# mirams/PyHillFit

Measured on AMD Instinct MI355X. Metric: MCMC samples/sec (whole node), higher is better.
Workload: dtype f64

## Files before the change

### pyhillfit_amd/csrc/phf_model.h

```cpp
#ifndef PHF_MODEL_H
#define PHF_MODEL_H

#include "phf_math.h"
#include "phf_philox.h"

#define PHF_SIGMA_FLOOR 1e-3
#define PHF_PIC50_RATE 0.2
#define PHF_PIC50_LOWER (-3.0)
#define PHF_HILL_UPPER 10.0
#define PHF_SIGMA_LOC 1e-3
#define PHF_SIGMA_SHAPE_M1 4.0
#define PHF_SIGMA_INV_SCALE (4.0 / (6.0 - 1e-3))
#define PHF_HILL_ARG_CAP 40.0

PHF_HD double phf_hill_den(int model, double ln_conc, double hill, double ln_ic50, phf_ktab k_exp) {
  const double a = (model == 1) ? (ln_conc - ln_ic50) : hill * (ln_conc - ln_ic50);
  return 1.0 + phf_exp_capped_k(__builtin_fmin(a, PHF_HILL_ARG_CAP), k_exp);
}

PHF_HD double phf_hill_percent(double w, phf_ktab k_exp) { return phf_fma(-PHF_K100(k_exp), w, PHF_K100(k_exp)); }
#define PHF_PCT_(w_) phf_hill_percent((w_), k_exp)

PHF_HD double phf_censored_z(double pred, double y, double inv_s) {
  const double sgn = (y > 50.0) ? 1.0 : -1.0;
  return (sgn * (pred - y)) * inv_s;
}

PHF_HD void phf_sl_log_target(int model, const double* lc, const double* y, const double* w, int n_other, int n_cens,
                              double n_other_points, double ss_within, double pi_bit, double temperature,
                              const double* th, phf_ktab k_exp, phf_ktab k_log,
                              double* out_lik, double* out_prior, double* out_ll1) {
  const double pic50 = th[0];
  const double hill = (model == 1) ? 1.0 : th[1];
  const double sigma = (model == 1) ? th[1] : th[2];
  const double ln_ic50 = PHF_LN10 * (6.0 - pic50);
  const double sl = sigma - PHF_SIGMA_LOC;
  const double inv_s = phf_rcp(sigma);
  const double log_sigma = phf_log_pos_k(sigma, k_log);
  const double log_sl = phf_log_pos_k(sl, k_log);

  double sse = ss_within, cens = 0.0;
  int j = 0;
  for (; j + 4 <= n_other; j += 4) {
    const phf_ktab ke = k_exp;
    const double d0 = phf_hill_den(model, lc[j], hill, ln_ic50, ke), d1 = phf_hill_den(model, lc[j + 1], hill, ln_ic50, ke);
    const double d2 = phf_hill_den(model, lc[j + 2], hill, ln_ic50, ke), d3 = phf_hill_den(model, lc[j + 3], hill, ln_ic50, ke);
    const double p01 = d0 * d1, p23 = d2 * d3;
    const double inv = phf_rcp(p01 * p23);
    const double i01 = inv * p23, i23 = inv * p01;
    const double r0 = y[j] - PHF_PCT_(i01 * d1), r1 = y[j + 1] - PHF_PCT_(i01 * d0);
    const double r2 = y[j + 2] - PHF_PCT_(i23 * d3), r3 = y[j + 3] - PHF_PCT_(i23 * d2);
    sse = phf_fma(w[j] * r0, r0, sse); sse = phf_fma(w[j + 1] * r1, r1, sse);
    sse = phf_fma(w[j + 2] * r2, r2, sse); sse = phf_fma(w[j + 3] * r3, r3, sse);
  }
  const int rem = n_other - j;
  if (rem == 3) {
    const phf_ktab ke = k_exp;
    const double d0 = phf_hill_den(model, lc[j], hill, ln_ic50, ke), d1 = phf_hill_den(model, lc[j + 1], hill, ln_ic50, ke);
    const double d2 = phf_hill_den(model, lc[j + 2], hill, ln_ic50, ke);
    const double p01 = d0 * d1;
    const double inv = phf_rcp(p01 * d2);
    const double i01 = inv * d2;
    const double r0 = y[j] - PHF_PCT_(i01 * d1), r1 = y[j + 1] - PHF_PCT_(i01 * d0);
    const double r2 = y[j + 2] - PHF_PCT_(inv * p01);
    sse = phf_fma(w[j] * r0, r0, sse); sse = phf_fma(w[j + 1] * r1, r1, sse); sse = phf_fma(w[j + 2] * r2, r2, sse);
  } else if (rem == 2) {
    const phf_ktab ke = k_exp;
    const double d0 = phf_hill_den(model, lc[j], hill, ln_ic50, ke), d1 = phf_hill_den(model, lc[j + 1], hill, ln_ic50, ke);
    const double inv = phf_rcp(d0 * d1);
    const double r0 = y[j] - PHF_PCT_(inv * d1), r1 = y[j + 1] - PHF_PCT_(inv * d0);
    sse = phf_fma(w[j] * r0, r0, sse); sse = phf_fma(w[j + 1] * r1, r1, sse);
  } else if (rem == 1) {
    const double r = y[j] - PHF_PCT_(phf_rcp(phf_hill_den(model, lc[j], hill, ln_ic50, k_exp)));
    sse = phf_fma(w[j] * r, r, sse);
  }
  j = n_other;
  const int n = n_other + n_cens;
  for (; j + 2 <= n; j += 2) {
    const phf_ktab ke = k_exp;
    const double d0 = phf_hill_den(model, lc[j], hill, ln_ic50, ke), d1 = phf_hill_den(model, lc[j + 1], hill, ln_ic50, ke);
    const double inv = phf_rcp(d0 * d1);
    const double z0 = phf_censored_z(PHF_PCT_(inv * d1), y[j], inv_s);
    const double z1 = phf_censored_z(PHF_PCT_(inv * d0), y[j + 1], inv_s);
    cens = phf_fma(w[j], phf_log_ndtr_tab(z0, -z0 * PHF_INV_SQRT2), cens);
    cens = phf_fma(w[j + 1], phf_log_ndtr_tab(z1, -z1 * PHF_INV_SQRT2), cens);
  }
  for (; j < n; ++j) {
    const double pred = PHF_PCT_(phf_rcp(phf_hill_den(model, lc[j], hill, ln_ic50, k_exp)));
    const double z = phf_censored_z(pred, y[j], inv_s);
    cens = phf_fma(w[j], phf_log_ndtr_tab(z, -z * PHF_INV_SQRT2), cens);
  }
  double a = cens - pi_bit;
  a = phf_fma(-n_other_points, log_sigma, a);
  a = phf_fma(-sse, 0.5 * inv_s * inv_s, a);
  if (sigma <= PHF_SIGMA_FLOOR) a = -PHF_INF;
  double lik = temperature * a;
  if (temperature == 0.0) lik = 0.0;
  *out_lik = lik;
  *out_ll1 = a;

  const int outside = (pic50 < PHF_PIC50_LOWER)
                      | (sigma <= PHF_SIGMA_LOC)
                      | ((model == 2) & ((hill < 0.0) | (hill > PHF_HILL_UPPER)));
  const double g = phf_fma(PHF_SIGMA_SHAPE_M1, log_sl, -sl * PHF_SIGMA_INV_SCALE);
  const double lp = -PHF_PIC50_RATE * pic50 + g;
  *out_prior = outside ? -PHF_INF : lp;
}

#define PHF_SHARE_PUT_(jj, d_) do { if (share_mask) den_slot[(jj) * slot_stride] = (d_); } while (0)
#define PHF_CDEN_(jj) ((((share_mask) >> ((jj) - n_other)) & 1u) ? den_slot[den_off[(jj) - n_other]] \
                                                                 : phf_hill_den(model, lc[jj], hill, ln_ic50, k_exp))
PHF_HD void phf_sl_log_target_shared(int model, const double* lc, const double* y, const double* w, int n_other, int n_cens,
                                     double n_other_points, double ss_within, double pi_bit, double temperature,
                                     const double* th, phf_ktab k_exp, phf_ktab k_log,
                                     unsigned share_mask, const int* den_off, double* den_slot, int slot_stride,
                                     double* out_lik, double* out_prior, double* out_ll1) {
  const double pic50 = th[0];
  const double hill = (model == 1) ? 1.0 : th[1];
  const double sigma = (model == 1) ? th[1] : th[2];
  const double ln_ic50 = PHF_LN10 * (6.0 - pic50);
  const double sl = sigma - PHF_SIGMA_LOC;
  const double inv_s = phf_rcp(sigma);
  const double log_sigma = phf_log_pos_k(sigma, k_log);
  const double log_sl = phf_log_pos_k(sl, k_log);

  double sse = ss_within, cens = 0.0;
  int j = 0;
  for (; j + 4 <= n_other; j += 4) {
    const phf_ktab ke = k_exp;
    const double d0 = phf_hill_den(model, lc[j], hill, ln_ic50, ke), d1 = phf_hill_den(model, lc[j + 1], hill, ln_ic50, ke);
    const double d2 = phf_hill_den(model, lc[j + 2], hill, ln_ic50, ke), d3 = phf_hill_den(model, lc[j + 3], hill, ln_ic50, ke);
    PHF_SHARE_PUT_(j, d0); PHF_SHARE_PUT_(j + 1, d1); PHF_SHARE_PUT_(j + 2, d2); PHF_SHARE_PUT_(j + 3, d3);
    const double p01 = d0 * d1, p23 = d2 * d3;
    const double inv = phf_rcp(p01 * p23);
    const double i01 = inv * p23, i23 = inv * p01;
    const double r0 = y[j] - PHF_PCT_(i01 * d1), r1 = y[j + 1] - PHF_PCT_(i01 * d0);
    const double r2 = y[j + 2] - PHF_PCT_(i23 * d3), r3 = y[j + 3] - PHF_PCT_(i23 * d2);
    sse = phf_fma(w[j] * r0, r0, sse); sse = phf_fma(w[j + 1] * r1, r1, sse);
    sse = phf_fma(w[j + 2] * r2, r2, sse); sse = phf_fma(w[j + 3] * r3, r3, sse);
  }
  const int rem = n_other - j;
  if (rem == 3) {
    const phf_ktab ke = k_exp;
    const double d0 = phf_hill_den(model, lc[j], hill, ln_ic50, ke), d1 = phf_hill_den(model, lc[j + 1], hill, ln_ic50, ke);
    const double d2 = phf_hill_den(model, lc[j + 2], hill, ln_ic50, ke);
    PHF_SHARE_PUT_(j, d0); PHF_SHARE_PUT_(j + 1, d1); PHF_SHARE_PUT_(j + 2, d2);
    const double p01 = d0 * d1;
    const double inv = phf_rcp(p01 * d2);
    const double i01 = inv * d2;
    const double r0 = y[j] - PHF_PCT_(i01 * d1), r1 = y[j + 1] - PHF_PCT_(i01 * d0);
    const double r2 = y[j + 2] - PHF_PCT_(inv * p01);
    sse = phf_fma(w[j] * r0, r0, sse); sse = phf_fma(w[j + 1] * r1, r1, sse); sse = phf_fma(w[j + 2] * r2, r2, sse);
  } else if (rem == 2) {
    const phf_ktab ke = k_exp;
    const double d0 = phf_hill_den(model, lc[j], hill, ln_ic50, ke), d1 = phf_hill_den(model, lc[j + 1], hill, ln_ic50, ke);
    PHF_SHARE_PUT_(j, d0); PHF_SHARE_PUT_(j + 1, d1);
    const double inv = phf_rcp(d0 * d1);
    const double r0 = y[j] - PHF_PCT_(inv * d1), r1 = y[j + 1] - PHF_PCT_(inv * d0);
    sse = phf_fma(w[j] * r0, r0, sse); sse = phf_fma(w[j + 1] * r1, r1, sse);
  } else if (rem == 1) {
    const double d0 = phf_hill_den(model, lc[j], hill, ln_ic50, k_exp);
    PHF_SHARE_PUT_(j, d0);
    const double r = y[j] - PHF_PCT_(phf_rcp(d0));
    sse = phf_fma(w[j] * r, r, sse);
  }
  j = n_other;
  const int n = n_other + n_cens;
  for (; j + 2 <= n; j += 2) {
    const double d0 = PHF_CDEN_(j), d1 = PHF_CDEN_(j + 1);
    const double inv = phf_rcp(d0 * d1);
    const double z0 = phf_censored_z(PHF_PCT_(inv * d1), y[j], inv_s);
    const double z1 = phf_censored_z(PHF_PCT_(inv * d0), y[j + 1], inv_s);
    cens = phf_fma(w[j], phf_log_ndtr_tab(z0, -z0 * PHF_INV_SQRT2), cens);
    cens = phf_fma(w[j + 1], phf_log_ndtr_tab(z1, -z1 * PHF_INV_SQRT2), cens);
  }
  for (; j < n; ++j) {
    const double pred = PHF_PCT_(phf_rcp(PHF_CDEN_(j)));
    const double z = phf_censored_z(pred, y[j], inv_s);
    cens = phf_fma(w[j], phf_log_ndtr_tab(z, -z * PHF_INV_SQRT2), cens);
  }
  double a = cens - pi_bit;
  a = phf_fma(-n_other_points, log_sigma, a);
  a = phf_fma(-sse, 0.5 * inv_s * inv_s, a);
  if (sigma <= PHF_SIGMA_FLOOR) a = -PHF_INF;
  double lik = temperature * a;
  if (temperature == 0.0) lik = 0.0;
  *out_lik = lik;
  *out_ll1 = a;

  const int outside = (pic50 < PHF_PIC50_LOWER)
                      | (sigma <= PHF_SIGMA_LOC)
                      | ((model == 2) & ((hill < 0.0) | (hill > PHF_HILL_UPPER)));
  const double g = phf_fma(PHF_SIGMA_SHAPE_M1, log_sl, -sl * PHF_SIGMA_INV_SCALE);
  const double lp = -PHF_PIC50_RATE * pic50 + g;
  *out_prior = outside ? -PHF_INF : lp;
}
#undef PHF_SHARE_PUT_
#undef PHF_CDEN_

PHF_HD double phf_sl_log_prior(int model, const double* th, phf_ktab k_log) {
  const double pic50 = th[0];
  const double hill = (model == 1) ? 1.0 : th[1];
  const double sigma = (model == 1) ? th[1] : th[2];
  const double sl = sigma - PHF_SIGMA_LOC;
  const double log_sl = phf_log_pos_k(sl, k_log);
  const int outside = (pic50 < PHF_PIC50_LOWER)
                      | (sigma <= PHF_SIGMA_LOC)
                      | ((model == 2) & ((hill < 0.0) | (hill > PHF_HILL_UPPER)));
  const double g = phf_fma(PHF_SIGMA_SHAPE_M1, log_sl, -sl * PHF_SIGMA_INV_SCALE);
  const double lp = -PHF_PIC50_RATE * pic50 + g;
  return outside ? -PHF_INF : lp;
}

PHF_HD double phf_mh_draws(int d, uint32_t chain_id, uint32_t problem_id, uint32_t t, uint32_t seed_lo,
                           uint32_t seed_hi, phf_ktab k_log, double* z) {
  const phf_u32x4 b = phf_philox_mh(chain_id, problem_id, t, 0u, seed_lo, seed_hi);
  z[0] = phf_normal_u32(b.w[0]);
  z[1] = phf_normal_u32(b.w[1]);
  if (d == 2) {
    z[2] = 0.0;
    const double u = phf_uniform53(b.w[2], b.w[3]);
    const double log_u = phf_log_pos_k(u, k_log);
    return (u < PHF_DBL_MIN) ? -PHF_INF : log_u;
  }
  z[2] = phf_normal_u32(b.w[2]);
  return phf_log_pos_k(phf_unit_open32(b.w[3]), k_log);
}

PHF_HD uint32_t phf_mh_draws_w3(uint32_t chain_id, uint32_t problem_id, uint32_t t, uint32_t seed_lo, uint32_t seed_hi, double* z) {
  const phf_u32x4 b = phf_philox_mh(chain_id, problem_id, t, 0u, seed_lo, seed_hi);
  z[0] = phf_normal_u32(b.w[0]);
  z[1] = phf_normal_u32(b.w[1]);
  z[2] = phf_normal_u32(b.w[2]);
  return b.w[3];
}

#define PHF_ACCEPT_U32_BAND 0x1p18f
PHF_HD int phf_mh_accept_u32(double x, uint32_t w, phf_ktab k_log) {
#if defined(__HIP_DEVICE_COMPILE__)
  const float t = __builtin_amdgcn_exp2f(__builtin_fmaf((float)x, 0x1.715476p+0f, 32.0f));
  const float dw = (float)w - t;
  bool acc = dw < 0.0f;
  if (PHF_ANY_LANE(__builtin_fabsf(dw) <= PHF_ACCEPT_U32_BAND)) {
    const bool exact = phf_log_pos_k(phf_unit_open32(w), k_log) < x;
    acc = (__builtin_fabsf(dw) <= PHF_ACCEPT_U32_BAND) ? exact : acc;
  }
  return acc;
#else
  return phf_log_pos_k(phf_unit_open32(w), k_log) < x;
#endif
}

#endif
```

### pyhillfit_amd/csrc/phf_single_level.hip

```cpp
#include <hip/hip_runtime.h>

#include "../../include/pyhillfit_amd.h"
#include "phf_common.h"
#include "phf_hier3_isa.h"
#include "phf_model.h"

namespace {

constexpr int kBlock = 64;
thread_local int g_last_sl_kernel = 0;
constexpr int kQueuePoison = 0x40000000;
constexpr int kQueueMaxRounds = 16;
constexpr int kDenSlots = 4;
constexpr int kMaxShared = 4;

template <int MODEL> struct Dim { static constexpr int d = (MODEL == 1) ? 2 : 3; };

#ifndef PHF_CHOL_FUSED_PIVOT
#define PHF_CHOL_FUSED_PIVOT 1
#endif
template <int D>
__device__ __forceinline__ void chol_packed(const double* c, double* l) {
  double inv[D];
#pragma unroll
  for (int i = 0; i < D; ++i) {
#pragma unroll
    for (int j = 0; j <= i; ++j) {
      double s = c[i * (i + 1) / 2 + j];
#pragma unroll
      for (int k = 0; k < j; ++k) s = phf_fma(-l[i * (i + 1) / 2 + k], l[j * (j + 1) / 2 + k], s);
      if (i == j) {
        const bool pos = s > 0.0;
        double ir = 0.0;
#if PHF_CHOL_FUSED_PIVOT
        const double rs = (i + 1 < D) ? phf_sqrt_rcp_pos(s, &ir) : phf_sqrt_pos(s);
#else
        const double rs = phf_sqrt_pos(s);
        ir = phf_rcp(rs);
#endif
        const double r = pos ? rs : 0.0;
        l[i * (i + 1) / 2 + i] = r;
        inv[i] = pos ? ir : 0.0;
      } else {
        l[i * (i + 1) / 2 + j] = s * inv[j];
      }
    }
  }
}

struct AdvanceArgs {
  phf_points pts;
  phf_problems prob;
  phf_mh_config cfg;
  int64_t t_begin, t_end;
  double* state;
  double* rows;
  double* moments;
  int64_t moments_after;
  int32_t blocks_per_problem;
  int32_t* queue;
  int32_t quantum;
};

__device__ __forceinline__ void stage_points(const phf_points& pts, int pair, double* s_pts, int& n_other,
                                             int& n_zero, int& n_hundred) {
  const int32_t* cnt = pts.counts + 4 * pair;
  n_other = cnt[0]; n_zero = cnt[1]; n_hundred = cnt[2];
  const int n = n_other + n_zero + n_hundred;
  for (int j = threadIdx.x; j < n; j += kBlock) {
    s_pts[j] = pts.ln_conc[(size_t)pair * pts.stride + j];
    s_pts[pts.stride + j] = pts.response[(size_t)pair * pts.stride + j];
    s_pts[2 * pts.stride + j] = pts.weight[(size_t)pair * pts.stride + j];
  }
  __syncthreads();
}

template <int MODEL, bool MOMENTS, int KO, int KC, unsigned SHARE, bool LONE_WAVE>
__device__ __forceinline__ void advance_body(const AdvanceArgs& a, const double* s_pts, double* s_den, const int* den_off, int q,
                                             int c, int pair, int n_other_rt, int n_cens_rt, const int64_t t_begin, const int64_t t_end) {
  static_assert(SHARE == 0 || (KO >= 1 && KO <= kDenSlots && KC >= 1 && KC <= kMaxShared && (SHARE >> KC) == 0),
                "shared denominators need a straight-line body with at most kDenSlots uncensored entries");
  constexpr int D = Dim<MODEL>::d;
  constexpr int NTRI = D * (D + 1) / 2;
  const int C = a.prob.chains_per_problem;
  const int n_other = (KO >= 0) ? KO : n_other_rt;
  const int n_cens = (KC >= 0) ? KC : n_cens_rt;
  const double* lc = s_pts;
  const double* yv = s_pts + a.pts.stride;
  const double* wv = s_pts + 2 * a.pts.stride;
  const double pi_bit = a.pts.pi_bit[pair];
  const double n_other_points = a.pts.extra[2 * pair], ss_within = a.pts.extra[2 * pair + 1];
  const double temperature = a.prob.temperature[q];
  const uint32_t pid = a.prob.problem_id[q];
  const uint32_t cid = a.prob.chain_id_base + (a.prob.chain_offset ? a.prob.chain_offset[q] : 0u) + (uint32_t)c;
  uint32_t seed_lo = (uint32_t)a.cfg.seed, seed_hi = (uint32_t)(a.cfg.seed >> 32);
  if (!LONE_WAVE) { asm volatile("" : "+v"(seed_lo)); asm volatile("" : "+v"(seed_hi)); }
  const size_t nchains = (size_t)a.prob.num_problems * C;
  const size_t g = (size_t)q * C + c;

  double th[D], mean[D], cov[NTRI], L[NTRI];
  double* sp = a.state + g;
#pragma unroll
  for (int i = 0; i < D; ++i) th[i] = sp[(size_t)i * nchains];
  double lt = sp[(size_t)D * nchains];
#pragma unroll
  for (int i = 0; i < D; ++i) mean[i] = sp[(size_t)(D + 1 + i) * nchains];
#pragma unroll
  for (int i = 0; i < NTRI; ++i) cov[i] = sp[(size_t)(2 * D + 1 + i) * nchains];
  double loga = sp[(size_t)(2 * D + 1 + NTRI) * nchains];
  double nacc = sp[(size_t)(2 * D + 2 + NTRI) * nchains];
  double ll1 = sp[(size_t)(2 * D + 3 + NTRI) * nchains];
  PHF_KFETCH_V(k_exp, phf_k_exp, PHF_K_EXP_N);
  PHF_KFETCH_V(k_log, phf_k_log, PHF_K_LOG_N);
  chol_packed<D>(cov, L);
  double sc = phf_exp_fast_k(0.5 * loga, k_exp);

  double m1[D + 1], m2[D + 1], mll = 0.0;
  constexpr bool want_moments = MOMENTS;
  if (want_moments) {
#pragma unroll
    for (int i = 0; i <= D; ++i) {
      m1[i] = a.moments[(size_t)i * nchains + g];
      m2[i] = a.moments[(size_t)(D + 1 + i) * nchains + g];
    }
    mll = a.moments[(size_t)(2 * D + 2) * nchains + g];
  }

  const int thin = a.cfg.thinning;
  int until_save = thin - (int)(t_begin % thin);
  const bool save_rows = a.rows != nullptr;
  const size_t row_stride = (size_t)a.prob.num_problems * (D + 1) * C;
  double* out = a.rows + ((size_t)q * (D + 1)) * C + c + (size_t)(t_begin / thin - a.t_begin / thin) * row_stride;

  double z[3];
  double log_u = 0.0;
  uint32_t w_u = 0u;
  if constexpr (D == 3) w_u = phf_mh_draws_w3(cid, pid, (uint32_t)(t_begin + 1), seed_lo, seed_hi, z);
  else log_u = phf_mh_draws(D, cid, pid, (uint32_t)(t_begin + 1), seed_lo, seed_hi, k_log, z);
  const bool reset_mean = a.cfg.reset_mean_at_adapt_start != 0;
  for (int64_t t = t_begin + 1; t <= t_end; ++t) {
    double star[D];
#pragma unroll
    for (int i = 0; i < D; ++i) {
      double v = L[i * (i + 1) / 2 + i] * z[i];
#pragma unroll
      for (int k = i - 1; k >= 0; --k) v = phf_fma(L[i * (i + 1) / 2 + k], z[k], v);
      star[i] = phf_fma(sc, v, th[i]);
    }
    double lik_star, prior_star, ll1_star;
    phf_sl_log_target_shared(MODEL, lc, yv, wv, n_other, n_cens, n_other_points, ss_within, pi_bit, temperature, star, k_exp, k_log,
                             SHARE, den_off, s_den + threadIdx.x, kBlock, &lik_star, &prior_star, &ll1_star);
    const double lt_star = lik_star + prior_star;
    const bool acc = (D == 3) ? (bool)phf_mh_accept_u32(lt_star - lt, w_u, k_log) : log_u < lt_star - lt;
    if (acc) {
#pragma unroll
      for (int i = 0; i < D; ++i) th[i] = star[i];
      lt = lt_star;
      ll1 = ll1_star;
    }
    nacc += acc ? 1.0 : 0.0;
    const bool adapting = t > a.cfg.adapt_start;
    const bool reset_now = reset_mean && t == a.cfg.adapt_start;
    const double gs_tab = a.cfg.gamma[adapting ? t - a.cfg.adapt_start : 0];
    const double gs = adapting ? gs_tab : 0.0;
    const double omg = 1.0 - gs;
    const double gm = reset_now ? 1.0 : gs, omm = reset_now ? 0.0 : omg;
    {
      double v[D];
#pragma unroll
      for (int i = 0; i < D; ++i) v[i] = th[i] - mean[i];
#pragma unroll
      for (int i = 0; i < D; ++i)
#pragma unroll
        for (int j = 0; j <= i; ++j)
          cov[i * (i + 1) / 2 + j] = phf_fma(gs, v[i] * v[j], omg * cov[i * (i + 1) / 2 + j]);
#pragma unroll
      for (int i = 0; i < D; ++i) mean[i] = phf_fma(gm, th[i], omm * mean[i]);
      loga = phf_fma(gs, acc ? 0.75 : -0.25, loga);
    }
    double z_next[3];
    double log_u_next = 0.0;
    uint32_t w_u_next = 0u;
    if constexpr (D == 3) w_u_next = phf_mh_draws_w3(cid, pid, (uint32_t)(t + 1), seed_lo, seed_hi, z_next);
    else log_u_next = phf_mh_draws(D, cid, pid, (uint32_t)(t + 1), seed_lo, seed_hi, k_log, z_next);
    chol_packed<D>(cov, L);
    sc = phf_exp_fast_k(0.5 * loga, k_exp);
#pragma unroll
    for (int i = 0; i < 3; ++i) z[i] = z_next[i];
    log_u = log_u_next;
    w_u = w_u_next;
    if (--until_save == 0) {
      until_save = thin;
      if (save_rows) {
#pragma unroll
        for (int i = 0; i < D; ++i) out[(size_t)i * C] = th[i];
        out[(size_t)D * C] = lt;
        out += row_stride;
      }
      if (want_moments && t > a.moments_after) {
#pragma unroll
        for (int i = 0; i < D; ++i) { m1[i] += th[i]; m2[i] = phf_fma(th[i], th[i], m2[i]); }
        m1[D] += lt; m2[D] = phf_fma(lt, lt, m2[D]);
        mll += ll1;
      }
    }
  }

#pragma unroll
  for (int i = 0; i < D; ++i) sp[(size_t)i * nchains] = th[i];
  sp[(size_t)D * nchains] = lt;
#pragma unroll
  for (int i = 0; i < D; ++i) sp[(size_t)(D + 1 + i) * nchains] = mean[i];
#pragma unroll
  for (int i = 0; i < NTRI; ++i) sp[(size_t)(2 * D + 1 + i) * nchains] = cov[i];
  sp[(size_t)(2 * D + 1 + NTRI) * nchains] = loga;
  sp[(size_t)(2 * D + 2 + NTRI) * nchains] = nacc;
  sp[(size_t)(2 * D + 3 + NTRI) * nchains] = ll1;
  if (want_moments) {
#pragma unroll
    for (int i = 0; i <= D; ++i) {
      a.moments[(size_t)i * nchains + g] = m1[i];
      a.moments[(size_t)(D + 1 + i) * nchains + g] = m2[i];
    }
    a.moments[(size_t)(2 * D + 2) * nchains + g] = mll;
  }
}

#define PHF_BODY_(ko, kc, sh) \
  advance_body<MODEL, MOMENTS, ko, kc, sh, WPS == 1>(a, s_pts, s_den, den_off, q, c, pair, n_other, n_cens, t_begin, t_end)
#define PHF_SHAPE_CASE(ko, kc) case (ko) * 8 + (kc): PHF_BODY_(ko, kc, 0u); break;
#define PHF_SHAPE_CASE_SHARED(ko, kc, sh) \
  case (ko) * 8 + (kc): if ((share & (sh)) == (sh)) PHF_BODY_(ko, kc, sh); else PHF_BODY_(ko, kc, 0u); break;
#define PHF_SHAPE_ROW(ko) PHF_SHAPE_CASE(ko, 0) PHF_SHAPE_CASE(ko, 1) PHF_SHAPE_CASE(ko, 2) PHF_SHAPE_CASE(ko, 3) PHF_SHAPE_CASE(ko, 4)

__device__ __forceinline__ unsigned share_map(const double* s_pts, int n_other, int n_cens, int* den_off) {
  unsigned share = 0;
#pragma unroll
  for (int m = 0; m < kMaxShared; ++m) {
    den_off[m] = 0;
    if (m < n_cens && n_other <= kDenSlots) {
      const long long b = __double_as_longlong(s_pts[n_other + m]);
#pragma unroll
      for (int j = kDenSlots - 1; j >= 0; --j)
        if (j < n_other && __double_as_longlong(s_pts[j]) == b) { share |= 1u << m; den_off[m] = j * kBlock; }
    }
    den_off[m] = __builtin_amdgcn_readfirstlane(den_off[m]);
  }
  return __builtin_amdgcn_readfirstlane(share);
}

template <int MODEL, bool MOMENTS, int WPS>
__device__ __forceinline__ void run_block(const AdvanceArgs& a, double* s_pts, double* s_den, int block, const int64_t t_begin,
                                          const int64_t t_end) {
  const int slot = block / a.blocks_per_problem;
  const int chunk = block - slot * a.blocks_per_problem;
  const int q = a.prob.launch_order ? a.prob.launch_order[slot] : slot;
  const int c = chunk * kBlock + threadIdx.x;
  int n_other, n_zero, n_hundred;
  const int pair = a.prob.pair_index[q];
  stage_points(a.pts, pair, s_pts, n_other, n_zero, n_hundred);
  if (c >= a.prob.chains_per_problem) return;
  const int n_cens = n_zero + n_hundred;
  int den_off[kMaxShared];
  const unsigned share = share_map(s_pts, n_other, n_cens, den_off);
  if (n_other <= 5 && n_cens <= 4) {
    switch (n_other * 8 + n_cens) {
      PHF_SHAPE_CASE(0, 1) PHF_SHAPE_CASE(0, 2) PHF_SHAPE_CASE(0, 3) PHF_SHAPE_CASE(0, 4)
      PHF_SHAPE_CASE(1, 0) PHF_SHAPE_CASE(1, 1) PHF_SHAPE_CASE(1, 2) PHF_SHAPE_CASE(1, 3) PHF_SHAPE_CASE_SHARED(1, 4, 0x8u)
      PHF_SHAPE_CASE(2, 0) PHF_SHAPE_CASE_SHARED(2, 1, 0x1u) PHF_SHAPE_CASE_SHARED(2, 2, 0x3u) PHF_SHAPE_CASE_SHARED(2, 3, 0x4u)
      PHF_SHAPE_CASE_SHARED(2, 4, 0xcu)
      PHF_SHAPE_CASE(3, 0) PHF_SHAPE_CASE(3, 1) PHF_SHAPE_CASE_SHARED(3, 2, 0x2u) PHF_SHAPE_CASE_SHARED(3, 3, 0x6u)
      PHF_SHAPE_CASE_SHARED(3, 4, 0xeu)
      PHF_SHAPE_CASE(4, 0) PHF_SHAPE_CASE_SHARED(4, 1, 0x1u) PHF_SHAPE_CASE_SHARED(4, 2, 0x3u) PHF_SHAPE_CASE_SHARED(4, 3, 0x7u)
      PHF_SHAPE_CASE_SHARED(4, 4, 0xfu)
      PHF_SHAPE_ROW(5)
      default: PHF_BODY_(-1, -1, 0u); break;
    }
    return;
  }
  PHF_BODY_(-1, -1, 0u);
}

template <int MODEL, bool MOMENTS, int WPS>
__global__ __launch_bounds__(kBlock, WPS) void mh_advance_kernel(const AdvanceArgs a) {
  PHF_MATH_TABLES_TO_LDS();
  PHF_NORMAL_TABLE_TO_LDS();
  PHF_LOGPHI_TABLE_TO_LDS();
  extern __shared__ double s_pts[];
  __shared__ double s_den[kDenSlots * kBlock];
  const bool queued = a.queue != nullptr;
  const int nblocks = a.blocks_per_problem * a.prob.num_problems;
  const int total = queued ? nblocks * (int)((a.t_end - a.t_begin + a.quantum - 1) / a.quantum) : 0;
  for (;;) {
    int b = blockIdx.x, k = 0;
    int64_t t0 = a.t_begin, t1 = a.t_end;
    if (queued) {
      int task = 0;
      if (threadIdx.x == 0) task = atomicAdd(a.queue, 1);
      task = __builtin_amdgcn_readfirstlane(task);
      if (task >= total) break;
      k = task / nblocks; b = task - k * nblocks;
      if (k > 0) {
        int polls = 0;
        while (__hip_atomic_load(a.queue + 1 + b, __ATOMIC_RELAXED, __HIP_MEMORY_SCOPE_AGENT) < k) {
          __builtin_amdgcn_s_sleep(16);
          ++polls;
          const bool gave_up = polls > (1 << 24) ||
                               ((polls & 1023) == 0 && __hip_atomic_load(a.queue + 1 + nblocks, __ATOMIC_RELAXED, __HIP_MEMORY_SCOPE_AGENT) != 0);
          if (gave_up) {
            if (threadIdx.x == 0) {
              __hip_atomic_store(a.queue + 1 + nblocks, 1, __ATOMIC_RELAXED, __HIP_MEMORY_SCOPE_AGENT);
              __hip_atomic_store(a.queue, kQueuePoison, __ATOMIC_RELAXED, __HIP_MEMORY_SCOPE_AGENT);
            }
            return;
          }
        }
        __builtin_amdgcn_fence(__ATOMIC_ACQUIRE, "agent");
      }
      t0 = a.t_begin + (int64_t)k * a.quantum;
      t1 = (t0 + a.quantum < a.t_end) ? t0 + a.quantum : a.t_end;
    }
    run_block<MODEL, MOMENTS, WPS>(a, s_pts, s_den, b, t0, t1);
    if (!queued) break;
    __builtin_amdgcn_fence(__ATOMIC_RELEASE, "agent");
    asm volatile("s_waitcnt vmcnt(0)" ::: "memory");
    __syncthreads();
    if (threadIdx.x == 0) __hip_atomic_store(a.queue + 1 + b, k + 1, __ATOMIC_RELAXED, __HIP_MEMORY_SCOPE_AGENT);
  }
}

struct InitArgs {
  phf_points pts;
  phf_problems prob;
  int32_t cov_identity;
  double cov_scale;
  const double* theta0;
  double* state;
  double* row0;
  int32_t blocks_per_problem;
};

template <int MODEL>
__global__ __launch_bounds__(kBlock) void mh_init_kernel(const InitArgs a) {
  PHF_MATH_TABLES_TO_LDS();
  PHF_LOGPHI_TABLE_TO_LDS();
  constexpr int D = Dim<MODEL>::d;
  constexpr int NTRI = D * (D + 1) / 2;
  extern __shared__ double s_pts[];
  const int q = blockIdx.x / a.blocks_per_problem;
  const int chunk = blockIdx.x - q * a.blocks_per_problem;
  const int C = a.prob.chains_per_problem;
  const int c = chunk * kBlock + threadIdx.x;
  int n_other, n_zero, n_hundred;
  const int pair = a.prob.pair_index[q];
  stage_points(a.pts, pair, s_pts, n_other, n_zero, n_hundred);
  if (c >= C) return;
  const size_t nchains = (size_t)a.prob.num_problems * C;
  const size_t g = (size_t)q * C + c;
  double th[D];
#pragma unroll
  for (int i = 0; i < D; ++i) th[i] = a.theta0[(size_t)i * nchains + g];
  double lik0, prior0, ll10;
  PHF_KFETCH_V(k_exp, phf_k_exp, PHF_K_EXP_N);
  PHF_KFETCH_V(k_log, phf_k_log, PHF_K_LOG_N);
  phf_sl_log_target(MODEL, s_pts, s_pts + a.pts.stride, s_pts + 2 * a.pts.stride, n_other, n_zero + n_hundred,
                    a.pts.extra[2 * pair], a.pts.extra[2 * pair + 1], a.pts.pi_bit[pair], a.prob.temperature[q],
                    th, k_exp, k_log, &lik0, &prior0, &ll10);
  const double lt = lik0 + prior0;
  double* sp = a.state + g;
#pragma unroll
  for (int i = 0; i < D; ++i) { sp[(size_t)i * nchains] = th[i]; sp[(size_t)(D + 1 + i) * nchains] = th[i]; }
  sp[(size_t)D * nchains] = lt;
#pragma unroll
  for (int i = 0; i < D; ++i)
#pragma unroll
    for (int j = 0; j <= i; ++j)
      sp[(size_t)(2 * D + 1 + i * (i + 1) / 2 + j) * nchains] =
          (i != j) ? 0.0 : (a.cov_identity ? a.cov_scale : a.cov_scale * __builtin_fabs(th[i]));
  sp[(size_t)(2 * D + 1 + NTRI) * nchains] = 0.0;
  sp[(size_t)(2 * D + 2 + NTRI) * nchains] = 0.0;
  sp[(size_t)(2 * D + 3 + NTRI) * nchains] = ll10;
  if (a.row0) {
    double* o = a.row0 + ((size_t)q * (D + 1)) * C + c;
#pragma unroll
    for (int i = 0; i < D; ++i) o[(size_t)i * C] = th[i];
    o[(size_t)D * C] = lt;
  }
}

template <int MODEL>
__global__ __launch_bounds__(256) void log_target_kernel(const phf_points pts, int64_t m, const int32_t* pair_index,
                                                          const double* temperature, const double* theta,
                                                          double* out_lik, double* out_prior) {
  PHF_MATH_TABLES_TO_LDS();
  PHF_LOGPHI_TABLE_TO_LDS();
  constexpr int D = Dim<MODEL>::d;
  const int64_t i = (int64_t)blockIdx.x * 256 + threadIdx.x;
  if (i >= m) return;
  const int pair = pair_index[i];
  const int32_t* cnt = pts.counts + 4 * pair;
  double th[D];
#pragma unroll
  for (int k = 0; k < D; ++k) th[k] = theta[(size_t)k * m + i];
  double lik, prior, ll1;
  PHF_KFETCH_V(k_exp, phf_k_exp, PHF_K_EXP_N);
  PHF_KFETCH_V(k_log, phf_k_log, PHF_K_LOG_N);
  phf_sl_log_target(MODEL, pts.ln_conc + (size_t)pair * pts.stride, pts.response + (size_t)pair * pts.stride,
                    pts.weight + (size_t)pair * pts.stride, cnt[0], cnt[1] + cnt[2], pts.extra[2 * pair], pts.extra[2 * pair + 1],
                    pts.pi_bit[pair], temperature[i], th, k_exp, k_log, &lik, &prior, &ll1);
  if (out_lik) out_lik[i] = lik;
  if (out_prior) out_prior[i] = prior;
}

__global__ void debug_math_kernel(int fn, int64_t n, const double* in, double* out) {
  PHF_MATH_TABLES_TO_LDS();
  PHF_LOGPHI_TABLE_TO_LDS();
  PHF_ERFC_TABLE_TO_LDS();
  PHF_NORMAL_TABLE_TO_LDS();
  const int64_t i = (int64_t)blockIdx.x * blockDim.x + threadIdx.x;
  if (fn == 22) {
    if (2 * i + 1 >= n) return;
    PHF_KFETCH_V(k_log, phf_k_log, PHF_K_LOG_N);
    const double x = in[2 * i];
    const uint32_t w = (uint32_t)in[2 * i + 1];
    out[2 * i] = phf_mh_accept_u32(x, w, k_log) ? 1.0 : 0.0;
    out[2 * i + 1] = (phf_log_pos_k(phf_unit_open32(w), k_log) < x) ? 1.0 : 0.0;
    return;
  }
  if (i >= n) return;
  const double x = in[i];
  double r, s, c;
  switch (fn) {
    case 0: r = phf_exp(x); break;
    case 1: r = phf_log(x); break;
    case 2: r = phf_erfcx_nonneg(x); break;
    case 3: r = phf_log_ndtr(x); break;
    case 4: r = phf_ndtr(x); break;
    case 5: r = phf_sqrt(x); break;
    case 6: r = 1.0 / x; break;
    case 7: phf_sincos_2pi_u32((uint32_t)x, &s, &c); r = s; break;
    case 9: r = phf_exp_fast(x); break;
    case 10: r = phf_log_fast(x); break;
    case 11: r = phf_log_ndtr_nonpos(x); break;
    case 12: r = phf_rcp(x); break;
    case 13: r = phf_sqrt_pos(x); break;
    case 14: r = phf_div(PHF_LN10, x); break;
    case 15: r = phf_sqrt_nonneg(x); break;
    case 16: r = phf_div(x, PHF_LN10); break;
    case 17: r = phf_normal_u32((uint32_t)x); break;
    case 18: r = phf_log_ndtr_tab(x, -x * PHF_INV_SQRT2); break;
    case 19: r = phf_erfc_tab(x); break;
    case 20: (void)phf_sqrt_rcp_pos(x, &r); break;
    case 21: r = phf_sqrt_rcp_pos(x, &s); break;
    default: phf_sincos_2pi_u32((uint32_t)x, &s, &c); r = c; break;
  }
  out[i] = r;
}

template <int ROUNDS>
__global__ void debug_philox_kernel(int64_t n, const uint32_t* ck, uint32_t* out) {
  const int64_t i = (int64_t)blockIdx.x * blockDim.x + threadIdx.x;
  if (i >= n) return;
  const uint32_t* c = ck + 6 * i;
  const phf_u32x4 r = phf_philox4x32_r(ROUNDS, c[0], c[1], c[2], c[3], c[4], c[5]);
  for (int k = 0; k < 4; ++k) out[4 * i + k] = r.w[k];
}

int check_common(const phf_points* pts, const phf_problems* prob, int model) {
  if (!pts || !prob) return phf_fail(PHF_ERR_INVALID_ARGUMENT, "null points/problems");
  if (model != 1 && model != 2) return phf_fail(PHF_ERR_INVALID_ARGUMENT, "model must be 1 or 2");
  if (pts->num_pairs <= 0 || pts->stride <= 0 || !pts->ln_conc || !pts->response || !pts->weight || !pts->counts || !pts->pi_bit || !pts->extra)
    return phf_fail(PHF_ERR_INVALID_ARGUMENT, "incomplete phf_points");
  if (prob->num_problems <= 0 || prob->chains_per_problem <= 0 || !prob->pair_index || !prob->temperature || !prob->problem_id)
    return phf_fail(PHF_ERR_INVALID_ARGUMENT, "incomplete phf_problems");
  if ((size_t)pts->stride * 24 > 160 * 1024) return phf_fail(PHF_ERR_UNSUPPORTED, "pair does not fit in LDS");
  const int64_t bpp = (prob->chains_per_problem + kBlock - 1) / kBlock;
  if (bpp * prob->num_problems > 0x7fffffffLL) return phf_fail(PHF_ERR_UNSUPPORTED, "too many chains for one launch");
  return PHF_OK;
}

}

extern "C" {

int phf_version(void) { return PHF_ABI_VERSION; }
int phf_single_level_last_kernel(void) { return g_last_sl_kernel; }

int phf_single_level_state_size(int model) {
  if (model == 1) return 2 * 2 + 3 + 4;
  if (model == 2) return 2 * 3 + 6 + 4;
  return phf_fail(PHF_ERR_INVALID_ARGUMENT, "model must be 1 or 2");
}

int phf_single_level_init(const phf_points* pts, const phf_problems* prob, int model, int cov_identity,
                          double cov_scale, const double* theta0, double* state, double* row0, void* stream) {
  if (int rc = check_common(pts, prob, model)) return rc;
  if (!theta0 || !state) return phf_fail(PHF_ERR_INVALID_ARGUMENT, "null theta0/state");
  phf_forget_device_memory_verdicts();
  InitArgs a{*pts, *prob, cov_identity, cov_scale, theta0, state, row0, 0};
  a.blocks_per_problem = (prob->chains_per_problem + kBlock - 1) / kBlock;
  const dim3 grid((unsigned)(a.blocks_per_problem * prob->num_problems)), block(kBlock);
  const size_t lds = (size_t)pts->stride * 24;
  if (model == 1) hipLaunchKernelGGL(mh_init_kernel<1>, grid, block, lds, (hipStream_t)stream, a);
  else hipLaunchKernelGGL(mh_init_kernel<2>, grid, block, lds, (hipStream_t)stream, a);
  return phf_check_launch("phf_single_level_init");
}

static int advance_impl(const phf_points* pts, const phf_problems* prob, const phf_mh_config* cfg, int64_t t_begin, int64_t t_end,
                        double* state, double* rows, double* moments, int64_t moments_after, int32_t quantum, int32_t* queue,
                        void* stream) {
  if (!cfg) return phf_fail(PHF_ERR_INVALID_ARGUMENT, "null config");
  if (int rc = check_common(pts, prob, cfg->model)) return rc;
  if (!state) return phf_fail(PHF_ERR_INVALID_ARGUMENT, "null state");
  if (cfg->thinning <= 0) return phf_fail(PHF_ERR_INVALID_ARGUMENT, "thinning must be positive");
  if (t_begin < 0 || t_end < t_begin || t_end > 0xffffffffLL) return phf_fail(PHF_ERR_INVALID_ARGUMENT, "bad iteration range");
  if (prob->kernel_hint & ~48u)
    return phf_fail(PHF_ERR_INVALID_ARGUMENT, "kernel_hint of a single-level launch: bit 4 = the hipcc kernel, bit 5 = the gfx950 assembly build; the other bits must be 0");
  if (!cfg->gamma) return phf_fail(PHF_ERR_INVALID_ARGUMENT, "gamma table required (gamma[0] is read even before adaptation starts)");
  if (t_end == t_begin) return PHF_OK;
  if (int rc = phf_require_device_memory(state, "state")) return rc;
  if (int rc = phf_require_device_memory(moments, "moments")) return rc;
  if (int rc = phf_require_device_memory(queue, "queue workspace")) return rc;
  AdvanceArgs a{*pts, *prob, *cfg, t_begin, t_end, state, rows, moments, moments_after, 0, nullptr, 0};
  a.blocks_per_problem = (prob->chains_per_problem + kBlock - 1) / kBlock;
  const int64_t nblocks = (int64_t)a.blocks_per_problem * prob->num_problems;
  const size_t lds = (size_t)pts->stride * 24;
  const bool lone = nblocks <= phf_simd_count();
  hipStream_t s = (hipStream_t)stream;
  int64_t grid_blocks = nblocks;
  if (queue && quantum > 0) {
    const int64_t slots = 2 * phf_simd_count();
    const int64_t nquanta = (t_end - t_begin + quantum - 1) / quantum;
    if (nquanta * nblocks > 0x3fffffffLL) return phf_fail(PHF_ERR_UNSUPPORTED, "too many tasks for one queued launch");
    if (!lone && nquanta >= 2 && nblocks > slots && nblocks <= kQueueMaxRounds * slots) {
      if (hipMemsetAsync(queue, 0, (size_t)(1 + nblocks) * sizeof(int32_t), s) != hipSuccess) return phf_check_launch("phf_single_level_advance_queued (memset)");
      a.queue = queue; a.quantum = quantum;
      grid_blocks = slots;
    }
  }
  static const bool isa_on = [] { const char* e = getenv("PHF_SL_ISA"); return e && e[0] == '1' && e[1] == 0; }();
  if (cfg->model == 2 && !moments && !lone && (isa_on || (prob->kernel_hint & 32u)) && !(prob->kernel_hint & 16u) && pts->stride <= PHF_ISA_SL_MAX_STRIDE &&
      cfg->adapt_start >= 0 && t_end < 0xffffffffLL && nblocks <= 0x7fffffffLL && phf_sl3_isa_available()) {
    phf_sl3_isa_args g{};
    g.state = state; g.rows = rows; g.gamma = cfg->gamma;
    g.ln_conc = pts->ln_conc; g.response = pts->response; g.weight = pts->weight; g.counts = pts->counts; g.pi_bit = pts->pi_bit; g.extra = pts->extra;
    g.pair_index = prob->pair_index; g.temperature = prob->temperature; g.problem_id = prob->problem_id;
    g.launch_order = prob->launch_order; g.chain_offset = prob->chain_offset;
    g.t_begin = (uint32_t)t_begin; g.t_end = (uint32_t)t_end;
    g.adapt_start = (uint32_t)(cfg->adapt_start > 0xffffffffLL ? 0xffffffffLL : cfg->adapt_start);
    g.thinning = cfg->thinning; g.reset_mean = cfg->reset_mean_at_adapt_start != 0 ? 1u : 0u;
    g.chains = prob->chains_per_problem; g.num_problems = prob->num_problems; g.bpp = a.blocks_per_problem;
    g.bpp_magic = phf_isa_magic((uint32_t)a.blocks_per_problem); g.total_waves = (int32_t)nblocks;
    g.seed_lo = (uint32_t)cfg->seed; g.seed_hi = (uint32_t)(cfg->seed >> 32);
    g.chain_id_base = prob->chain_id_base; g.pts_stride = pts->stride;
    g.until_save0 = cfg->thinning - (int32_t)(t_begin % cfg->thinning);
    bool ok = true;
    if (a.queue) {
      const int64_t nquanta = (t_end - t_begin + a.quantum - 1) / a.quantum;
      ok = a.quantum % cfg->thinning == 0 && t_begin % cfg->thinning == 0 && nquanta * nblocks < (1LL << 31);
      g.queue = a.queue; g.quantum = (uint32_t)a.quantum; g.num_tasks = (int32_t)(nquanta * nblocks);
      g.blocks_magic = phf_isa_magic((uint32_t)nblocks); g.rows_per_quantum = (uint32_t)(a.quantum / cfg->thinning);
    }
    if (ok) {
      g_last_sl_kernel = a.queue ? 3 : 2;
      const int64_t isa_slots = 4LL * phf_simd_count();
      const int64_t grid_waves = a.queue ? (nblocks < isa_slots ? nblocks : isa_slots) : nblocks;
      return phf_sl3_isa_advance(&g, (int)grid_waves, s);
    }
  }
  g_last_sl_kernel = 1;
  const dim3 grid((unsigned)grid_blocks), block(kBlock);
#define PHF_LAUNCH_ADVANCE(M, MOM, W) hipLaunchKernelGGL((mh_advance_kernel<M, MOM, W>), grid, block, lds, s, a)
  if (cfg->model == 1) {
    if (moments) { if (lone) PHF_LAUNCH_ADVANCE(1, true, 1); else PHF_LAUNCH_ADVANCE(1, true, 2); }
    else { if (lone) PHF_LAUNCH_ADVANCE(1, false, 1); else PHF_LAUNCH_ADVANCE(1, false, 2); }
  } else {
    if (moments) { if (lone) PHF_LAUNCH_ADVANCE(2, true, 1); else PHF_LAUNCH_ADVANCE(2, true, 2); }
    else { if (lone) PHF_LAUNCH_ADVANCE(2, false, 1); else PHF_LAUNCH_ADVANCE(2, false, 2); }
  }
#undef PHF_LAUNCH_ADVANCE
  return phf_check_launch("phf_single_level_advance");
}

int phf_single_level_advance(const phf_points* pts, const phf_problems* prob, const phf_mh_config* cfg,
                             int64_t t_begin, int64_t t_end, double* state, double* rows, double* moments,
                             int64_t moments_after, void* stream) {
  return advance_impl(pts, prob, cfg, t_begin, t_end, state, rows, moments, moments_after, 0, nullptr, stream);
}

int phf_single_level_advance_queued(const phf_points* pts, const phf_problems* prob, const phf_mh_config* cfg,
                                    int64_t t_begin, int64_t t_end, double* state, double* rows, double* moments,
                                    int64_t moments_after, int32_t quantum, int32_t* queue, void* stream) {
  if (quantum <= 0 || !queue) return phf_fail(PHF_ERR_INVALID_ARGUMENT, "queued advance needs a positive quantum and a queue workspace");
  return advance_impl(pts, prob, cfg, t_begin, t_end, state, rows, moments, moments_after, quantum, queue, stream);
}

int phf_single_level_queue_status(const int32_t* queue, int64_t num_blocks, void* stream) {
  if (!queue || num_blocks <= 0) return phf_fail(PHF_ERR_INVALID_ARGUMENT, "bad arguments to phf_single_level_queue_status");
  int32_t fault = 0;
  if (hipMemcpyAsync(&fault, queue + 1 + num_blocks, sizeof(fault), hipMemcpyDeviceToHost, (hipStream_t)stream) != hipSuccess ||
      hipStreamSynchronize((hipStream_t)stream) != hipSuccess)
    return phf_check_launch("phf_single_level_queue_status");
  if (fault != 0)
    return phf_fail(PHF_ERR_DRAINED, "a queued single-level launch drained (a wavefront's wait for its block's previous quantum did not end): "
                                     "states, rows and moments written since are stale");
  return PHF_OK;
}

int phf_single_level_log_target(const phf_points* pts, int model, int64_t m, const int32_t* pair_index,
                                const double* temperature, const double* theta, double* out_lik,
                                double* out_prior, void* stream) {
  if (!pts || (model != 1 && model != 2) || m < 0 || !pair_index || !temperature || !theta)
    return phf_fail(PHF_ERR_INVALID_ARGUMENT, "bad arguments to phf_single_level_log_target");
  if (m == 0) return PHF_OK;
  const dim3 grid((unsigned)((m + 255) / 256)), block(256);
  if (model == 1) hipLaunchKernelGGL(log_target_kernel<1>, grid, block, 0, (hipStream_t)stream, *pts, m, pair_index, temperature, theta, out_lik, out_prior);
  else hipLaunchKernelGGL(log_target_kernel<2>, grid, block, 0, (hipStream_t)stream, *pts, m, pair_index, temperature, theta, out_lik, out_prior);
  return phf_check_launch("phf_single_level_log_target");
}

int phf_debug_math(int fn, int64_t n, const double* in, double* out, void* stream) {
  if (fn < 0 || fn > 22 || n < 0 || (fn == 22 && n % 2) || !in || !out) return phf_fail(PHF_ERR_INVALID_ARGUMENT, "bad arguments to phf_debug_math");
  if (n == 0) return PHF_OK;
  hipLaunchKernelGGL(debug_math_kernel, dim3((unsigned)((n + 255) / 256)), dim3(256), 0, (hipStream_t)stream, fn, n, in, out);
  return phf_check_launch("phf_debug_math");
}

int phf_philox_rounds(void) { return PHF_PHILOX_ROUNDS; }

int phf_debug_philox_rounds(int rounds, int64_t n, const uint32_t* counter_key, uint32_t* out, void* stream) {
  if ((rounds != 7 && rounds != 10) || n < 0 || !counter_key || !out) return phf_fail(PHF_ERR_INVALID_ARGUMENT, "bad arguments to phf_debug_philox_rounds (rounds: 7 or 10)");
  if (n == 0) return PHF_OK;
  const dim3 grid((unsigned)((n + 255) / 256)), block(256);
  if (rounds == 7) hipLaunchKernelGGL(debug_philox_kernel<7>, grid, block, 0, (hipStream_t)stream, n, counter_key, out);
  else hipLaunchKernelGGL(debug_philox_kernel<10>, grid, block, 0, (hipStream_t)stream, n, counter_key, out);
  return phf_check_launch("phf_debug_philox_rounds");
}

int phf_debug_philox(int64_t n, const uint32_t* counter_key, uint32_t* out, void* stream) {
  return phf_debug_philox_rounds(PHF_PHILOX_ROUNDS, n, counter_key, out, stream);
}

}
```

Before: 73.34 billion.

## Use branch-free fast Cholesky with wave-uniform fallback and precomputed adaptation schedule

Replaces the per-pivot positivity selects in the inner-loop Cholesky with a fast path that only accumulates an all-positive flag, falling back to the guarded version when any lane in the wave sees a non-positive pivot. The MCMC loop is rewritten around a 32-bit iteration counter, with the adaptation start and mean-reset step precomputed before the loop. The gamma lookup goes through a constant address-space pointer and is prefetched one iteration ahead. This is meant to cut per-iteration ALU and branch work in the hot loop. In exchange it adds a wave-wide vote and a possible second Cholesky when any lane sees a degenerate covariance.

```diff
diff --git a/pyhillfit_amd/csrc/phf_model.h b/pyhillfit_amd/csrc/phf_model.h
--- a/pyhillfit_amd/csrc/phf_model.h
+++ b/pyhillfit_amd/csrc/phf_model.h
@@ -12,6 +12,12 @@
 #define PHF_SIGMA_SHAPE_M1 4.0
 #define PHF_SIGMA_INV_SCALE (4.0 / (6.0 - 1e-3))
 #define PHF_HILL_ARG_CAP 40.0
+
+#if defined(__HIP_DEVICE_COMPILE__)
+#define PHF_RARE_PATH(x) __asm__("" : "+v"(x))
+#else
+#define PHF_RARE_PATH(x) ((void)0)
+#endif
 
 PHF_HD double phf_hill_den(int model, double ln_conc, double hill, double ln_ic50, phf_ktab k_exp) {
   const double a = (model == 1) ? (ln_conc - ln_ic50) : hill * (ln_conc - ln_ic50);
diff --git a/pyhillfit_amd/csrc/phf_single_level.hip b/pyhillfit_amd/csrc/phf_single_level.hip
--- a/pyhillfit_amd/csrc/phf_single_level.hip
+++ b/pyhillfit_amd/csrc/phf_single_level.hip
@@ -46,6 +46,41 @@
       }
     }
   }
+}
+
+template <int D>
+__device__ __forceinline__ bool chol_packed_fast(const double* c, double* l) {
+  double inv[D];
+  bool all_pos = true;
+#pragma unroll
+  for (int i = 0; i < D; ++i) {
+#pragma unroll
+    for (int j = 0; j <= i; ++j) {
+      double s = c[i * (i + 1) / 2 + j];
+#pragma unroll
+      for (int k = 0; k < j; ++k) s = phf_fma(-l[i * (i + 1) / 2 + k], l[j * (j + 1) / 2 + k], s);
+      if (i == j) {
+        all_pos &= s > 0.0;
+        double ir = 0.0;
+#if PHF_CHOL_FUSED_PIVOT
+        l[i * (i + 1) / 2 + i] = (i + 1 < D) ? phf_sqrt_rcp_pos(s, &ir) : phf_sqrt_pos(s);
+#else
+        l[i * (i + 1) / 2 + i] = phf_sqrt_pos(s);
+        ir = phf_rcp(l[i * (i + 1) / 2 + i]);
+#endif
+        inv[i] = ir;
+      } else {
+        l[i * (i + 1) / 2 + j] = s * inv[j];
+      }
+    }
+  }
+  return all_pos;
+}
+
+template <int D>
+__device__ __forceinline__ void chol_packed_rare_select(const double* c, double* l) {
+  const bool all_pos = chol_packed_fast<D>(c, l);
+  if (PHF_ANY_LANE(!all_pos)) chol_packed<D>(c, l);
 }
 
 struct AdvanceArgs {
@@ -112,7 +147,7 @@
   double ll1 = sp[(size_t)(2 * D + 3 + NTRI) * nchains];
   PHF_KFETCH_V(k_exp, phf_k_exp, PHF_K_EXP_N);
   PHF_KFETCH_V(k_log, phf_k_log, PHF_K_LOG_N);
-  chol_packed<D>(cov, L);
+  chol_packed_rare_select<D>(cov, L);
   double sc = phf_exp_fast_k(0.5 * loga, k_exp);
 
   double m1[D + 1], m2[D + 1], mll = 0.0;
@@ -137,8 +172,19 @@
   uint32_t w_u = 0u;
   if constexpr (D == 3) w_u = phf_mh_draws_w3(cid, pid, (uint32_t)(t_begin + 1), seed_lo, seed_hi, z);
   else log_u = phf_mh_draws(D, cid, pid, (uint32_t)(t_begin + 1), seed_lo, seed_hi, k_log, z);
-  const bool reset_mean = a.cfg.reset_mean_at_adapt_start != 0;
-  for (int64_t t = t_begin + 1; t <= t_end; ++t) {
+  const uint32_t n_iter = (uint32_t)(t_end - t_begin);
+  const int64_t ahead = a.cfg.adapt_start - t_begin;
+  const uint32_t idle = ahead <= 0 ? 0u : (ahead >= (int64_t)n_iter ? n_iter : (uint32_t)ahead);
+  const uint32_t reset_i = (a.cfg.reset_mean_at_adapt_start != 0 && ahead >= 1 && ahead <= (int64_t)n_iter) ? (uint32_t)ahead : 0u;
+  const __attribute__((address_space(4))) double* gamma_k = (const __attribute__((address_space(4))) double*)a.cfg.gamma;
+  const auto gamma_of = [&](uint32_t i) {
+    const bool on = i > idle && i - 1u < n_iter;
+    const double g = gamma_k[on ? (int64_t)i - ahead : (int64_t)0];
+    return on ? g : 0.0;
+  };
+  double gs = gamma_of(1u);
+  for (uint32_t it = 1; it - 1u < n_iter; ++it) {
+    const int64_t t = t_begin + it;
     double star[D];
 #pragma unroll
     for (int i = 0; i < D; ++i) {
@@ -159,12 +205,12 @@
       ll1 = ll1_star;
     }
     nacc += acc ? 1.0 : 0.0;
-    const bool adapting = t > a.cfg.adapt_start;
-    const bool reset_now = reset_mean && t == a.cfg.adapt_start;
-    const double gs_tab = a.cfg.gamma[adapting ? t - a.cfg.adapt_start : 0];
-    const double gs = adapting ? gs_tab : 0.0;
     const double omg = 1.0 - gs;
-    const double gm = reset_now ? 1.0 : gs, omm = reset_now ? 0.0 : omg;
+    double gm = gs, omm = omg;
+    if (it == reset_i) {
+      gm = 1.0; omm = 0.0;
+      PHF_RARE_PATH(omm);
+    }
     {
       double v[D];
 #pragma unroll
@@ -183,7 +229,8 @@
     uint32_t w_u_next = 0u;
     if constexpr (D == 3) w_u_next = phf_mh_draws_w3(cid, pid, (uint32_t)(t + 1), seed_lo, seed_hi, z_next);
     else log_u_next = phf_mh_draws(D, cid, pid, (uint32_t)(t + 1), seed_lo, seed_hi, k_log, z_next);
-    chol_packed<D>(cov, L);
+    gs = gamma_of(it + 1u);
+    chol_packed_rare_select<D>(cov, L);
     sc = phf_exp_fast_k(0.5 * loga, k_exp);
 #pragma unroll
     for (int i = 0; i < 3; ++i) z[i] = z_next[i];
```

New measurement: 75.92 billion, median of 6. +3.5%, better.
